# pxl-th/SLAM.jl

Measured on AMD Instinct MI355X. Metric: frames/sec KITTI-05 stereo @1k kpts; local-BA ms/iter for 50-KF window, higher is better.
Workload: dtype f64

## Files before the change

### slam.jl_amd/csrc/kpset.hip

```cpp
#include "kpset.hpp"
#include <algorithm>
#include "geom_device.hpp"
#include "work_order.hpp"
#include "kf_host.hpp"
#include <cmath>
#include <type_traits>

#define WORK_BAND_PX 16
#define KPSET_SORT_LDS_BYTES 65536
static int work_band() { static const int band = [] { const char *v = getenv("SLAMHIP_WORK_BAND"); const int b = v ? atoi(v) : WORK_BAND_PX; return b < 0 ? 0 : b; }(); return band; }
struct WorkOrder { int H, W, band, pad; };
#define SEL_NAME(k) k
#define SEL_ARG
#define SEL_STREAM(b) b
#define SEL_STREAMS(S) S
#define SEL_SELF(s) s
#include "kpset_kernels.inc"
#undef SEL_NAME
#undef SEL_ARG
#undef SEL_STREAM
#undef SEL_STREAMS
#undef SEL_SELF
#define SEL_NAME(k) k##_sel
#define SEL_ARG , const int *sel
#define SEL_STREAM(b) sel[b]
#define SEL_STREAMS(S) (int)gridDim.x
#define SEL_SELF(s) (int)blockIdx.x
#include "kpset_kernels.inc"
#undef SEL_NAME
#undef SEL_ARG
#undef SEL_STREAM
#undef SEL_STREAMS
#undef SEL_SELF

int kpset_build_worklist(slam_ctx *ctx, slam_kpset *ks, int H, int W, bool selected)
{
    WorkOrder O;
    O.H = H; O.W = W; O.pad = ks->sort_pad; O.band = H > 0 && W > 0 && ks->sort_pad > 0 ? work_band() : 0;
    const size_t lds = O.band > 0 ? (size_t)ks->sort_pad * 8 : 0;
    if (selected && ks->n_sel != KPSEL_ALL)
        hipLaunchKernelGGL(k_kpset_worklist_sel, dim3(ks->n_sel), dim3(256), lds, ctx->stream, (const int *)ks->v.count, ks->S, ks->v.cap, ks->work, ks->ntot, (const double *)ks->v.yx, O,
                           (const int *)ks->sel_idx);
    else
        hipLaunchKernelGGL(k_kpset_worklist, dim3(ks->S), dim3(256), lds, ctx->stream, (const int *)ks->v.count, ks->S, ks->v.cap, ks->work, ks->ntot, (const double *)ks->v.yx, O);
    HIP_TRY(ctx, hipGetLastError());
    return SLAM_OK;
}

int kpset_stage_params(slam_ctx *ctx, slam_kpset *ks, const double *host, size_t n, const double **dev_out)
{
    const size_t slot_d = (size_t)ks->S * KP_PAR;
    ARG_TRY(ctx, n <= slot_d);
    const int sl = ks->par_slot; ks->par_slot = (sl + 1) & 7;
    HIP_TRY(ctx, hipEventSynchronize(ks->par_ev[sl]));
    double *h = ks->par_host + (size_t)sl * slot_d, *dv = ks->par + (size_t)sl * slot_d;
    memcpy(h, host, n * 8);
    HIP_TRY(ctx, hipMemcpyAsync(dv, h, n * 8, hipMemcpyHostToDevice, ctx->stream));
    HIP_TRY(ctx, hipEventRecord(ks->par_ev[sl], ctx->stream));
    *dev_out = dv;
    return SLAM_OK;
}

int kpset_compact(slam_ctx *ctx, slam_kpset *ks, int mode, const uint8_t *flags_dev, bool selected)
{
    if (selected && ks->n_sel != KPSEL_ALL)
        hipLaunchKernelGGL(k_kpset_compact_sel, dim3(ks->n_sel), dim3(256), 0, ctx->stream, ks->v, mode, flags_dev, (const int *)ks->sel_idx);
    else
        hipLaunchKernelGGL(k_kpset_compact, dim3(ks->S), dim3(256), 0, ctx->stream, ks->v, mode, flags_dev);
    HIP_TRY(ctx, hipGetLastError());
    return SLAM_OK;
}

struct KTriArgs {
    TwoViewMats M;
    const double *Twc;
    double max_error, min_depth;
};
__device__ __forceinline__ void k_kpset_triangulate_slot(const KpsetView &K, const KTriArgs &T, const int *work, int i)
{
    const size_t q = (size_t)work[i];
    if (!K.stereo[q] || K.is3d[q]) return;
    const int s = (int)(q / K.cap);
    const double x1 = K.yx[2 * q + 1], y1 = K.yx[2 * q], x2 = K.syx[2 * q + 1], y2 = K.syx[2 * q];
    double L[4];
    dlt_two_view(x1, y1, x2, y2, T.M.P1, T.M.P2, L);
    const bool ok = two_view_gates(L, T.M.T21, T.M.cam1, T.M.cam2, x1, y1, x2, y2, T.max_error, T.min_depth, true);
    if (ok) {
        const double *W = T.Twc + 16 * (size_t)s;
        for (int r = 0; r < 3; r++) K.xyz[3 * q + r] = ((W[r] * L[0] + W[r + 4] * L[1]) + W[r + 8] * L[2]) + W[r + 12] * L[3];
        K.is3d[q] = 1;
    } else K.stereo[q] = 0;
}
__global__ __launch_bounds__(64) void k_kpset_triangulate(KpsetView K, KTriArgs T, const int *work, const int *ntot)
{
    const int n = ntot[0];
    for (int i = blockIdx.x * 64 + threadIdx.x; i < n; i += gridDim.x * 64) k_kpset_triangulate_slot(K, T, work, i);
}

struct KTempArgs {
    const double *par;
    const double *tab;
    const int *kf_cur, *kf_lo; int nkf;
    double max_error, min_depth, min_parallax;
    uint8_t *flags;
};
__device__ __forceinline__ void k_kpset_tri_temporal_slot(const KpsetView &K, const KTempArgs &T, const int *work, int i)
{
    const size_t q = (size_t)work[i];
    if (K.is3d[q] || !K.haskf[q]) return;
    const int s = (int)(q / K.cap), kf = K.fkf[q];
    if (kf == T.kf_cur[s] || kf < T.kf_lo[s]) return;
    const double *par = T.par + KP_PAR * (size_t)s, *cam = par + KP_PAR_CAM, *dist = par + KP_PAR_DIST;
    const double *E = T.tab + ((size_t)s * T.nkf + (kf % T.nkf)) * 64;
    const double *P2 = E, *T21 = E + 16, *REL = E + 32, *WOB = E + 48;
    const double fx = cam[0], fy = cam[1], cx = cam[2], cy = cam[3];
    double y1, x1, y2, x2, qy, qx;
    undistort_px(cam, dist, K.fyx[2 * q], K.fyx[2 * q + 1], y1, x1);
    undistort_px(cam, dist, K.yx[2 * q], K.yx[2 * q + 1], y2, x2);
    rotate_project<4>(REL, cam, (x2 - cx) / fx, (y2 - cy) / fy, qy, qx);
    const double pdy = y1 - qy, pdx = x1 - qx;
    const bool gated = sqrt(pdy * pdy + pdx * pdx) > T.min_parallax;
    const double P1[16] = {fx, 0, 0, 0, 0, fy, 0, 0, cx, cy, 1, 0, 0, 0, 0, 1};
    double L[4];
    dlt_two_view(x1, y1, x2, y2, P1, P2, L);
    const bool ok = two_view_gates(L, T21, cam, cam, x1, y1, x2, y2, T.max_error, T.min_depth, gated);
    if (ok) {
        for (int r = 0; r < 3; r++) K.xyz[3 * q + r] = ((WOB[r] * L[0] + WOB[r + 4] * L[1]) + WOB[r + 8] * L[2]) + WOB[r + 12] * L[3];
// ... 90 lines not shown
    double cam[4], dist[4];
    load_cam(par, cam, dist);
    const double fx = cam[0], fy = cam[1], cx = cam[2], cy = cam[3];
    const bool comp = (A.flags & 1) != 0, only2d = (A.flags & 2) != 0;
    for (int w = tid; w < A.words; w += 256) s_bits[w] = 0;
    if (tid == 0) s_base = 0;
    int c[4] = {0, 0, 0, 0};
    for (int j = tid; j < n; j += 256) {
        const bool f3 = A.is3d[b + j] != 0, fk = A.haskf[b + j] != 0;
        c[0] += f3; c[1] += A.stereo[b + j] != 0; c[2] += fk; c[3] += fk && !(only2d && f3);
    }
    kf_block_sum4(c, s_c);
    const int m = c[3];
    const bool in_lds = m <= KF_TERMS_LDS;
    unsigned long long *gterm = A.terms ? A.terms + b : nullptr;
    const double ylim = (double)A.gr * (double)A.cell, xlim = (double)A.gc * (double)A.cell, low = -(double)A.cell;
    double psum = 0.0;
    int isnan_any = 0;
    for (int c0 = 0; c0 < n; c0 += 256) {
        const int j = c0 + tid;
        bool take = false;
        double y = 0.0, x = 0.0;
        if (j < n) {
            y = A.yx[2 * (b + j)]; x = A.yx[2 * (b + j) + 1];
            const double ry = rint(y), rx = rint(x);
            if (ry > low && ry < ylim && rx > low && rx < xlim) {
                const int cell = ((int)ry / A.cell) * A.gc + (int)rx / A.cell;
                atomicOr(&s_bits[cell >> 5], 1u << (cell & 31));
            }
            take = A.haskf[b + j] != 0 && !(only2d && A.is3d[b + j] != 0);
        }
        const int pos = ordered_slot(take, s_w, &s_base);
        if (take) {
            const size_t q = b + j;
            double uy, ux, vy, vx, qy, qx, t;
            undistort_px(cam, dist, y, x, uy, ux);
            undistort_px(cam, dist, A.kyx[2 * q], A.kyx[2 * q + 1], vy, vx);
            if (comp) {
                rotate_project<3>(par, cam, (ux - cx) / fx, (uy - cy) / fy, qy, qx);
                const double dy = qy - vy, dx = qx - vx;
                t = sqrt(dy * dy + dx * dx);
            } else {
                const double dy = uy - vy, dx = ux - vx;
                t = sqrt(dy * dy + dx * dx);
            }
            psum += t;
            isnan_any |= t != t;
            const unsigned long long bits = (unsigned long long)__double_as_longlong(t);
            if (in_lds) s_term[pos] = bits; else gterm[pos] = bits;
        }
    }
    for (int o = 32; o > 0; o >>= 1) psum += __shfl_xor(psum, o, 64);
    if (lane == 0) s_par[wv] = psum;
    __threadfence_block();
    const int has_nan = __syncthreads_or(isnan_any);
    int occ[4] = {0, 0, 0, 0};
    for (int w = tid; w < A.words; w += 256) occ[0] += __popc(s_bits[w]);
    kf_block_sum4(occ, s_c);
    double median = 0.0;
    if (m > 0) {
        if (has_nan) median = __longlong_as_double(0x7FF8000000000000ll);
        else median = in_lds ? kf_median(s_term, m, s_hist, s_w, s_sel, s_min) : kf_median(gterm, m, s_hist, s_w, s_sel, s_min);
    }
    if (tid == 0) {
        double *o = A.out + SLAM_KF_STATS * (size_t)z;
        o[KF_N] = (double)n; o[KF_N3D] = (double)c[0]; o[KF_NSTEREO] = (double)c[1]; o[KF_NHASKF] = (double)c[2]; o[KF_CELLS] = (double)occ[0]; o[KF_NPAR] = (double)m;
        o[KF_MEAN] = m > 0 ? ((s_par[0] + s_par[1]) + (s_par[2] + s_par[3])) / (double)m : 0.0;
        o[KF_MEDIAN] = median;
    }
}

static size_t kpset_regions(slam_kpset *ks, char *base)
{
    Layout Lo;
    auto region = [&](auto *&p, size_t bytes) { const size_t at = Lo.take(bytes); if (base) p = (std::remove_reference_t<decltype(p)>)(base + at); };
    KpsetView &v = ks->v;
    const size_t S = (size_t)ks->S, n = S * v.cap;
    region(v.yx, n * 16); region(v.oyx, n * 16); region(v.syx, n * 16); region(v.xyz, n * 24); region(v.id, n * 8);
    region(v.is3d, n); region(v.stereo, n); region(v.st, n); region(v.count, S * 4); region(ks->work, n * 4); region(ks->ntot, 64);
    region(ks->next_id, S * 8); region(ks->par, 8 * S * KP_PAR * 8); region(v.kyx, n * 16); region(v.haskf, n); region(v.fyx, n * 16);
    region(v.fkf, n * 4); region(v.kfcount, S * 4);
    region(ks->sel_idx, S * 4 + S);
    if (base) ks->sel_mask = (uint8_t *)(ks->sel_idx + S);
    return Lo.size();
}

struct KpField { void *dev; size_t bytes; const void *host; };
static int kpset_copy(slam_ctx *ctx, const slam_kpset *ks, int s, int n, hipMemcpyKind kind, bool wait, std::initializer_list<KpField> fields)
{
    if (n <= 0) return SLAM_OK;
    for (const KpField &f : fields) {
        if (!f.host) continue;
        void *d = (char *)f.dev + (size_t)s * ks->v.cap * f.bytes, *h = const_cast<void *>(f.host);
        HIP_TRY(ctx, hipMemcpyAsync(kind == hipMemcpyHostToDevice ? d : h, kind == hipMemcpyHostToDevice ? h : d, (size_t)n * f.bytes, kind, ctx->stream));
    }
    if (wait) HIP_TRY(ctx, slam_stream_wait(ctx->stream));
    return SLAM_OK;
}
static int kpset_download_begin(slam_ctx *ctx, slam_kpset *ks, int s, const char *who, int cap_out, int *n_out, bool with_kf, int *kf_count)
{
    HIP_TRY(ctx, hipSetDevice(ctx->device));
    int n = 0, kc = 0;
    HIP_TRY(ctx, hipMemcpyAsync(&n, ks->v.count + s, 4, hipMemcpyDeviceToHost, ctx->stream));
    if (with_kf) HIP_TRY(ctx, hipMemcpyAsync(&kc, ks->v.kfcount + s, 4, hipMemcpyDeviceToHost, ctx->stream));
    HIP_TRY(ctx, slam_stream_wait(ctx->stream));
    *n_out = n; if (kf_count) *kf_count = kc;
    if (n > cap_out) return slam_fail(ctx, SLAM_ERR_CAPACITY, "%s: %d keypoints but cap = %d", who, n, cap_out);
    return SLAM_OK;
}

int kpset_read_back(slam_ctx *ctx, char *h, std::initializer_list<KpReadBack> parts)
{
    for (const KpReadBack &p : parts) HIP_TRY(ctx, hipMemcpyAsync(h + p.at, p.dev, p.bytes, hipMemcpyDeviceToHost, ctx->stream));
    HIP_TRY(ctx, slam_stream_wait(ctx->stream));
    for (const KpReadBack &p : parts) if (p.out) memcpy(p.out, h + p.at, p.bytes);
    return SLAM_OK;
}

extern "C" {

int slam_kpset_destroy(slam_kpset *ks);

int slam_kpset_create(slam_ctx *ctx, int S, int cap, slam_kpset **out)
{
    ARG_TRY(ctx, ctx != nullptr && out != nullptr && S >= 1 && S <= 128 && cap >= 1 && (size_t)S * cap < (1u << 30));
    HIP_TRY(ctx, hipSetDevice(ctx->device));
    slam_kpset *ks = new slam_kpset();
    ks->device = ctx->device; ks->S = S; ks->v.cap = cap;
    const size_t bytes = kpset_regions(ks, nullptr);
    { size_t pad = 1; while (pad < (size_t)cap) pad <<= 1; ks->sort_pad = work_band() > 0 && pad * 8 <= KPSET_SORT_LDS_BYTES ? (int)pad : 0; }
    hipError_t e = hipMalloc((void **)&ks->base, bytes);
    if (e == hipSuccess) e = hipMemsetAsync(ks->base, 0, bytes, ctx->stream);
    if (e == hipSuccess) e = slam_stream_wait(ctx->stream);
    if (e != hipSuccess) { if (ks->base) (void)hipFree(ks->base); delete ks; return slam_fail(ctx, SLAM_ERR_HIP, "slam_kpset_create: %s", hipGetErrorString(e)); }
    kpset_regions(ks, ks->base);
    e = hipHostMalloc((void **)&ks->par_host, (size_t)8 * S * KP_PAR * 8);
    for (int i = 0; i < 8 && e == hipSuccess; i++) { e = hipEventCreateWithFlags(&ks->par_ev[i], hipEventDisableTiming); if (e == hipSuccess) e = hipEventRecord(ks->par_ev[i], ctx->stream); }
    if (e != hipSuccess) { slam_kpset_destroy(ks); return slam_fail(ctx, SLAM_ERR_HIP, "slam_kpset_create: %s", hipGetErrorString(e)); }
    *out = ks;
    return SLAM_OK;
}

int slam_kpset_destroy(slam_kpset *ks)
{
    if (!ks) return SLAM_OK;
    (void)hipSetDevice(ks->device);
    (void)hipDeviceSynchronize();
    if (ks->base) (void)hipFree(ks->base);
    if (ks->par_host) (void)hipHostFree(ks->par_host);
    if (ks->kf_stats) (void)hipFree(ks->kf_stats);
    if (ks->kf_terms) (void)hipFree(ks->kf_terms);
    for (int i = 0; i < 8; i++) if (ks->par_ev[i]) (void)hipEventDestroy(ks->par_ev[i]);
    if (ks->sel_pin) (void)hipHostFree(ks->sel_pin);
    for (int i = 0; i < 8; i++) if (ks->sel_ev[i]) (void)hipEventDestroy(ks->sel_ev[i]);
    delete ks;
    return SLAM_OK;
}

int slamhip_test_kpset_worklist(slam_ctx *ctx, slam_kpset *ks, int H, int W, int *work_out, int *ntot_out, int *band_out)
{
    ARG_TRY(ctx, ctx != nullptr && ks != nullptr && work_out != nullptr && ntot_out != nullptr && band_out != nullptr);
    HIP_TRY(ctx, hipSetDevice(ctx->device));
    int rc = kpset_build_worklist(ctx, ks, H, W);
    if (rc) return rc;
    HIP_TRY(ctx, hipMemcpyAsync(work_out, ks->work, (size_t)ks->S * ks->v.cap * 4, hipMemcpyDeviceToHost, ctx->stream));
    HIP_TRY(ctx, hipMemcpyAsync(ntot_out, ks->ntot, 4, hipMemcpyDeviceToHost, ctx->stream));
// ... 233 lines not shown
```

### slam.jl_amd/csrc/kpset.hpp

```cpp
#pragma once
#include "common.hpp"
#include "kpset_select.hpp"
#include <initializer_list>

struct KpsetView {
    double *yx;
    double *oyx;
    double *syx;
    double *xyz;
    double *kyx;
    double *fyx;
    int64_t *id;
    uint8_t *is3d, *stereo, *st, *haskf;
    int *fkf;
    int *kfcount;
    int *count;
    int cap;
};

constexpr int KP_PAR = 32, KP_PAR_CAM = 16, KP_PAR_DIST = 20, KP_PAR_SHIFT = 24;
__device__ __forceinline__ void load_cam(const double *par, double *cam, double *dist) { for (int k = 0; k < 4; k++) { cam[k] = par[KP_PAR_CAM + k]; dist[k] = par[KP_PAR_DIST + k]; } }

struct slam_kpset {
    int device = 0, S = 0;
    char *base = nullptr;
    KpsetView v = {};
    int *work = nullptr;
    int sort_pad = 0;
    int *ntot = nullptr;
    int64_t *next_id = nullptr;
    double *par = nullptr, *par_host = nullptr;
    hipEvent_t par_ev[8] = {};
    int par_slot = 0;
    double *kf_stats = nullptr;
    unsigned long long *kf_terms = nullptr;
    int n_sel = KPSEL_ALL;
    int *sel_idx = nullptr; uint8_t *sel_mask = nullptr;
    uint8_t sel_host[128] = {};
    char *sel_pin = nullptr;
    hipEvent_t sel_ev[8] = {};
    int sel_slot = 0;
};

int kpset_stage_params(slam_ctx *ctx, slam_kpset *ks, const double *host, size_t n, const double **dev_out);
int kpset_build_worklist(slam_ctx *ctx, slam_kpset *ks, int H, int W, bool selected = false);
int kpset_compact(slam_ctx *ctx, slam_kpset *ks, int mode, const uint8_t *flags_dev, bool selected = false);
inline bool kpset_none_selected(const slam_kpset *ks) { return ks->n_sel == 0; }
inline int kpset_sel_streams(const slam_kpset *ks) { return kpset_select_streams(ks->S, ks->n_sel); }
inline const int *kpset_sel_table(const slam_kpset *ks) { return ks->n_sel == KPSEL_ALL ? nullptr : ks->sel_idx; }
inline int kpset_grid_bound(const slam_kpset *ks, int n_bound) { const int nmax = ks->S * ks->v.cap; return n_bound > 0 && n_bound < nmax ? n_bound : nmax; }
inline int kpset_sel_grid_bound(const slam_kpset *ks, int n_bound) { return kpset_select_bound(ks->S, ks->v.cap, ks->n_sel, n_bound); }
struct KpReadBack { size_t at; const void *dev; size_t bytes; void *out; };
int kpset_read_back(slam_ctx *ctx, char *h, std::initializer_list<KpReadBack> parts);
```

### slam.jl_amd/csrc/kpset_kernels.inc

```

__global__ __launch_bounds__(256) void SEL_NAME(k_kpset_worklist)(const int *count, int S, int cap, int *work, int *ntot, const double *yx, WorkOrder O SEL_ARG)
{
    extern __shared__ unsigned long long s_word[];
    const int s = SEL_STREAM(blockIdx.x), tid = threadIdx.x, lane = tid & 63;
    int off = 0, t = 0;
    for (int i = lane; i < SEL_STREAMS(S); i += 64) { const int v = count[SEL_STREAM(i)]; t += v; off += i < SEL_SELF(s) ? v : 0; }
#pragma unroll
    for (int m = 32; m >= 1; m >>= 1) { off += __shfl_xor(off, m); t += __shfl_xor(t, m); }
    if (SEL_SELF(s) == 0 && tid == 0) ntot[0] = t;
    const int n = count[s];
    if (O.band <= 0 || n > O.pad) {
        for (int j = tid; j < n; j += 256) work[off + j] = s * cap + j;
        return;
    }
    int P = 1;
    while (P < n) P <<= 1;
    const double *p = yx + 2 * (size_t)s * cap;
    for (int j = tid; j < P; j += 256)
        s_word[j] = j < n ? ((unsigned long long)work_key(p[2 * j], p[2 * j + 1], O.H, O.W, O.band) << 32) | (unsigned)j : ~0ull;
    __syncthreads();
    for (int k = 2; k <= P; k <<= 1)
        for (int d = k >> 1; d > 0; d >>= 1) {
            for (int u = tid; u < (P >> 1); u += 256) {
                const int i = ((u & ~(d - 1)) << 1) | (u & (d - 1));
                const unsigned long long a = s_word[i], c = s_word[i + d];
                if ((a > c) == ((i & k) == 0)) { s_word[i] = c; s_word[i + d] = a; }
            }
            __syncthreads();
        }
    for (int j = tid; j < n; j += 256) work[off + j] = s * cap + (int)(unsigned)s_word[j];
}

__global__ __launch_bounds__(256) void SEL_NAME(k_kpset_compact)(KpsetView K, int mode, const uint8_t *flags SEL_ARG)
{
    __shared__ int s_w[4], s_base;
    const int s = SEL_STREAM(blockIdx.x), tid = threadIdx.x, lane = tid & 63, wv = tid >> 6;
    const size_t b = (size_t)s * K.cap;
    const int n = K.count[s];
    if (tid == 0) s_base = 0;
    __syncthreads();
    for (int c0 = 0; c0 < n; c0 += 256) {
        const int j = c0 + tid;
        bool keep = false;
        double y = 0, x = 0, sy = 0, sx = 0, X0 = 0, X1 = 0, X2 = 0, ky = 0, kx = 0, fy0 = 0, fx0 = 0; int64_t id = 0; uint8_t f3 = 0, fs = 0, fk = 0; int fkid = 0;
        if (j < n) {
            const size_t q = b + j;
            if (mode == 0) { const uint8_t t = K.st[q]; keep = t != 0; if (t == 1) { y = K.oyx[2 * q]; x = K.oyx[2 * q + 1]; } else { y = K.yx[2 * q]; x = K.yx[2 * q + 1]; } }
            else { keep = flags[q] == 0; y = K.yx[2 * q]; x = K.yx[2 * q + 1]; }
            if (keep) { sy = K.syx[2 * q]; sx = K.syx[2 * q + 1]; X0 = K.xyz[3 * q]; X1 = K.xyz[3 * q + 1]; X2 = K.xyz[3 * q + 2]; id = K.id[q]; f3 = K.is3d[q]; fs = K.stereo[q];
                        ky = K.kyx[2 * q]; kx = K.kyx[2 * q + 1]; fk = K.haskf[q]; fy0 = K.fyx[2 * q]; fx0 = K.fyx[2 * q + 1]; fkid = K.fkf[q]; }
        }
        const unsigned long long m = __ballot(keep);
        const int rank = __builtin_popcountll(m & ((1ull << lane) - 1ull));
        if (lane == 0) s_w[wv] = __builtin_popcountll(m);
        __syncthreads();
        int wbase = 0;
        for (int i = 0; i < wv; i++) wbase += s_w[i];
        const int total = s_w[0] + s_w[1] + s_w[2] + s_w[3];
        if (keep) {
            const size_t q = b + s_base + wbase + rank;
            K.yx[2 * q] = y; K.yx[2 * q + 1] = x; K.syx[2 * q] = sy; K.syx[2 * q + 1] = sx;
            K.xyz[3 * q] = X0; K.xyz[3 * q + 1] = X1; K.xyz[3 * q + 2] = X2; K.id[q] = id; K.is3d[q] = f3; K.stereo[q] = fs;
            K.kyx[2 * q] = ky; K.kyx[2 * q + 1] = kx; K.haskf[q] = fk; K.fyx[2 * q] = fy0; K.fyx[2 * q + 1] = fx0; K.fkf[q] = fkid;
        }
        __syncthreads();
        if (tid == 0) s_base += total;
        __syncthreads();
    }
    if (tid == 0) K.count[s] = s_base;
}

extern "C" __global__ __launch_bounds__(256) void SEL_NAME(k_kpset_keyframe)(KpsetView K SEL_ARG)
{
    const int s = SEL_STREAM(blockIdx.y), j = blockIdx.x * 256 + threadIdx.x;
    if (j >= K.count[s]) return;
    const size_t q = (size_t)s * K.cap + j;
    const double y = K.yx[2 * q], x = K.yx[2 * q + 1];
    if (!K.haskf[q]) { K.fyx[2 * q] = y; K.fyx[2 * q + 1] = x; K.fkf[q] = K.kfcount[s]; }
    K.kyx[2 * q] = y; K.kyx[2 * q + 1] = x; K.haskf[q] = 1;
}
```

### slam.jl_amd/csrc/lk.hip

```cpp
#include "kpset.hpp"
#include "geom_device.hpp"
#include "work_order.hpp"
#include <vector>
#include <cmath>
#include <cstdlib>
#include <type_traits>

struct LKTune {
    int pyramid_levels, levels3d, window, iterations;
    double eig_thr, eps, max_distance;
    bool nonneg() const { return pyramid_levels >= 0 && levels3d >= 0 && window >= 0 && iterations >= 0; }
};
struct LKArgs {
    PyrView prev, cur;
    const double *pts, *disp0;
    int n;
    LKTune tune;
    double *out;
    uint8_t *status;
};

#ifdef LK_TRACE
__device__ unsigned long long g_lk_ticks[8];
#define LKT_BEGIN unsigned long long _t0 = wall_clock64()
// ... 318 lines not shown
    double qy = py, qx = px, cy = dy, cx = dx;
    for (int k = 0; k <= pyramid_levels + 1; k++) {
        const bool back = k == pyramid_levels + 1;
        const int level = back ? 1 : pyramid_levels + 1 - k;
        if (back) {
            ny = py + cy; nx = px + cx;
            qy = ny; qx = nx;
            cy = -cy * 1.0; cx = -cx * 1.0;
        }
        const PyrView *pf = back ? &cur : &prev, *ps = back ? &prev : &cur;
        const bool ok = lk_level<LK_MAXE, TOL>(shifted(pf->lv[level - 1], back ? offC : offP), shifted(ps->lv[level - 1], back ? offP : offC),
                                          level, qy, qx, cy, cx, t.window, t.iterations, t.eig_thr, back ? 1e-2 : t.eps);
        if (!ok) return false;
    }
    const double b0 = ny + cy, b1 = nx + cx;
    const double d0 = py - b0, d1 = px - b1;
    return !(sqrt(d0 * d0 + d1 * d1) >= t.max_distance);
}

#define LK_XCDS 8
__device__ __forceinline__ int xcd_point(int n)
{
    const int per = (n + LK_XCDS - 1) / LK_XCDS;
    return (int)(blockIdx.x % LK_XCDS) * per + (int)(blockIdx.x / LK_XCDS);
}
static inline unsigned lk_grid(int n) { return (unsigned)((n + LK_XCDS - 1) / LK_XCDS) * LK_XCDS; }

template <int LK_MAXE>
__global__ __launch_bounds__(64) LK_OCC void k_fb_track(LKArgs A)
{
    const int i = xcd_point(A.n);
    if (i >= A.n) return;
    const double py = A.pts[2 * i], px = A.pts[2 * i + 1];
    const double dy = A.disp0 ? A.disp0[2 * i] : 0.0, dx = A.disp0 ? A.disp0[2 * i + 1] : 0.0;
    double ny = nan(""), nx = nan("");
    const bool ok = fb_point<LK_MAXE>(A.prev, A.cur, py, px, dy, dx, A.tune, A.tune.pyramid_levels, ny, nx);
    if ((threadIdx.x & 63) == 0) {
        A.out[2 * i] = ny; A.out[2 * i + 1] = nx;
        A.status[i] = ok ? 1 : 0;
    }
}

struct FlowArgs {
    LKArgs lk;
    const uint8_t *is3d; const double *proj;
    const int *img;
    size_t zs_from, zs_to;
};
template <int LK_MAXE>
__global__ __launch_bounds__(64) LK_OCC void k_flow_match(FlowArgs F)
{
    const LKArgs &A = F.lk;
    const int i = xcd_point(A.n);
    if (i >= A.n) return;
    LKT_BEGIN;
    const double py = A.pts[2 * i], px = A.pts[2 * i + 1];
    double ny = nan(""), nx = nan("");
    bool ok = false;
    const size_t zi = F.img ? (size_t)F.img[i] : 0;
    const size_t offP = zi * F.zs_from, offC = zi * F.zs_to;
    for (int att = F.is3d[i] ? 0 : 1; att < 2 && !ok; att++) {
        double dy = 0.0, dx = 0.0;
        if (att == 0) {
            const double scale = 1.0 / (double)(1 << A.tune.levels3d);
            dy = scale * (F.proj[2 * i] - py); dx = scale * (F.proj[2 * i + 1] - px);
        }
        ok = fb_point<LK_MAXE>(A.prev, A.cur, py, px, dy, dx, A.tune, att == 0 ? A.tune.levels3d : A.tune.pyramid_levels, ny, nx, offP, offC);
    }
    LKT(0);
    if ((threadIdx.x & 63) == 0) {
        A.out[2 * i] = ok ? ny : nan(""); A.out[2 * i + 1] = ok ? nx : nan("");
        A.status[i] = ok ? 1 : 0;
    }
}

struct KpMatchArgs {
    PyrView from, to; size_t zs_from, zs_to;
    LKTune tune;
    double *yx, *oyx, *syx; const double *xyz; const uint8_t *is3d; uint8_t *st, *stereo; int cap;
    const int *work, *ntot;
    int prior;
    const double *par;
    int H, W, stereo_mode; double epipolar;
};
template <int LK_MAXE, bool TOL>
__global__ __launch_bounds__(64) LK_OCC void k_kpset_match(KpMatchArgs M)
{
    const int ntot = M.ntot[0], per = (ntot + LK_XCDS - 1) / LK_XCDS;
    for (int slotx = (int)(blockIdx.x / LK_XCDS); slotx < per; slotx += (int)(gridDim.x / LK_XCDS)) {
    const int idx = (int)(blockIdx.x % LK_XCDS) * per + slotx;
    if (idx >= ntot) break;
    const size_t q = (size_t)M.work[idx];
    const int s = (int)(q / M.cap);
    const double *P = M.par + KP_PAR * (size_t)s, *cam = P + KP_PAR_CAM, *dist = P + KP_PAR_DIST;
    const double py = M.yx[2 * q], px = M.yx[2 * q + 1];
    const bool is3 = M.is3d[q] != 0;
    double pry = py, prx = px;
    if (is3) {
        if (M.prior == 1) {
            const double X0 = M.xyz[3 * q], X1 = M.xyz[3 * q + 1], X2 = M.xyz[3 * q + 2];
            const double cx = ((P[0] * X0 + P[4] * X1) + P[8] * X2) + P[12];
            const double cy = ((P[1] * X0 + P[5] * X1) + P[9] * X2) + P[13];
            const double cz = ((P[2] * X0 + P[6] * X1) + P[10] * X2) + P[14];
            pdn_to_pixel(cam, dist, cy / cz, cx / cz, pry, prx);
        } else if (M.prior == 2) { pry = py + P[KP_PAR_SHIFT]; prx = px + P[KP_PAR_SHIFT + 1]; }
    }
    const bool inside = 1 <= pry && pry <= (double)M.H && 1 <= prx && prx <= (double)M.W;
    const bool lane0 = (threadIdx.x & 63) == 0;
    if (is3 && !inside) {
        if (lane0) { M.st[q] = M.stereo_mode ? 0 : 2; if (M.stereo_mode) M.stereo[q] = 0; }
        continue;
    }
    const size_t offF = (size_t)s * M.zs_from, offT = (size_t)s * M.zs_to;
    double ny = nan(""), nx = nan("");
    bool ok = false;
    for (int att = is3 ? 0 : 1; att < 2 && !ok; att++) {
        double dy = 0.0, dx = 0.0;
        if (att == 0) {
            const double scale = 1.0 / (double)(1 << M.tune.levels3d);
            dy = scale * (pry - py); dx = scale * (prx - px);
        }
        ok = fb_point<LK_MAXE, TOL>(M.from, M.to, py, px, dy, dx, M.tune, att == 0 ? M.tune.levels3d : M.tune.pyramid_levels, ny, nx, offF, offT);
    }
    if (lane0 && !M.stereo_mode) {
        M.oyx[2 * q] = ok ? ny : nan(""); M.oyx[2 * q + 1] = ok ? nx : nan("");
        M.st[q] = ok ? 1 : 0;
    } else if (lane0) {
        if (ok) {
            double uy, ux;
            undistort_px(cam, dist, ny, nx, uy, ux);
            if (fabs(py - uy) > M.epipolar) ok = false;
        }
        if (ok) { M.syx[2 * q] = py; M.syx[2 * q + 1] = nx; }
        M.stereo[q] = ok ? 1 : 0;
        M.st[q] = 2;
    }
    }
}

template <class F> static void lk_launch(int window, F f)
{
    switch (lk_slots(window)) {
    case 3: f(std::integral_constant<int, 3>{}); break;
    case 6: f(std::integral_constant<int, 6>{}); break;
    default: f(std::integral_constant<int, 9>{});
    }
}

static int match_check(slam_ctx *ctx, const slam_pyr *from, const slam_pyr *to, const LKTune &t)
{
    const int need = t.pyramid_levels > t.levels3d ? t.pyramid_levels : t.levels3d;
    if (!(from->levels > need && to->levels > need)) return slam_fail(ctx, SLAM_ERR_LAYERS, "Not enough layers in pyramids.");
    ARG_TRY(ctx, from->H[0] == to->H[0] && from->W[0] == to->W[0]);
    if (from->target_only) return slam_fail(ctx, SLAM_ERR_ARG, "the source pyramid of a match was updated with SLAM_PYR_TARGET_ONLY: its gradient planes exist at level 0 only");
    return SLAM_OK;
}

static int kpset_match(slam_ctx *ctx, slam_kpset *ks, const slam_pyr *from0, const slam_pyr *to0, const double *params,
                       int prior, const LKTune &t, int stereo_mode, double epipolar, int n_bound)
{
    ARG_TRY(ctx, ctx != nullptr && ks != nullptr && from0 != nullptr && to0 != nullptr);
    ARG_TRY(ctx, from0->batch_index == 0 && to0->batch_index == 0 && from0->batch_size >= ks->S && to0->batch_size >= ks->S);
    ARG_TRY(ctx, t.nonneg() && prior >= 0 && prior <= 2 && (prior == 0 || params != nullptr));
    int rc = match_check(ctx, from0, to0, t);
    if (rc) return rc;
    HIP_TRY(ctx, hipSetDevice(ctx->device));
    const bool selected = stereo_mode != 0;
    if (selected && kpset_none_selected(ks)) return SLAM_OK;
    KpMatchArgs M;
    M.from = from0->view; M.to = to0->view; M.zs_from = from0->zstride; M.zs_to = to0->zstride;
    M.tune = t;
    const KpsetView &v = ks->v;
    M.yx = v.yx; M.oyx = v.oyx; M.syx = v.syx; M.xyz = v.xyz; M.is3d = v.is3d; M.st = v.st; M.stereo = v.stereo; M.cap = v.cap;
    M.work = ks->work; M.ntot = ks->ntot; M.prior = prior; M.H = from0->H[0]; M.W = from0->W[0]; M.stereo_mode = stereo_mode; M.epipolar = epipolar;
    std::vector<double> zero;
    if (!params) { zero.assign((size_t)ks->S * KP_PAR, 0.0); for (int s = 0; s < ks->S; s++) { zero[KP_PAR * s + KP_PAR_CAM] = zero[KP_PAR * s + KP_PAR_CAM + 1] = 1.0; } params = zero.data(); }
    rc = kpset_stage_params(ctx, ks, params, (size_t)ks->S * KP_PAR, &M.par);
    if (rc) return rc;
    rc = kpset_build_worklist(ctx, ks, M.H, M.W, selected);
    if (rc) return rc;
    int nb = selected ? kpset_sel_grid_bound(ks, n_bound) : kpset_grid_bound(ks, n_bound);
    static const int grid_cap = [] { const char *v = getenv("SLAMHIP_LK_GRID"); return v ? atoi(v) : 0; }();
    if (grid_cap > 0 && nb > grid_cap) nb = grid_cap;
    { ProfScope span(ctx, "fb_track");
      static const bool no_tol_lk = getenv("SLAMHIP_NO_TOL_LK") != nullptr;
      const bool tol = from0->tol_planes && to0->tol_planes && !no_tol_lk;
      if (tol) lk_launch(t.window, [&](auto N) { hipLaunchKernelGGL((k_kpset_match<N.value, true>), dim3(lk_grid(nb)), dim3(64), 0, ctx->stream, M); });
      else lk_launch(t.window, [&](auto N) { hipLaunchKernelGGL((k_kpset_match<N.value, false>), dim3(lk_grid(nb)), dim3(64), 0, ctx->stream, M); }); }
    HIP_TRY(ctx, hipGetLastError());
    return kpset_compact(ctx, ks, 0, nullptr, selected);
}

extern "C" int slam_kpset_flow_match(slam_ctx *ctx, slam_kpset *ks, const slam_pyr *from0, const slam_pyr *to0, const double *params, int prior,
                                     int pyramid_levels, int pyramid_levels_3d, int window, int iterations, double eig_thr, double eps,
                                     double max_distance, int n_bound)
{
    return kpset_match(ctx, ks, from0, to0, params, prior, {pyramid_levels, pyramid_levels_3d, window, iterations, eig_thr, eps, max_distance}, 0, 0.0, n_bound);
}
extern "C" int slam_kpset_stereo_match(slam_ctx *ctx, slam_kpset *ks, const slam_pyr *left0, const slam_pyr *right0, const double *params, int prior,
                                       int pyramid_levels, int pyramid_levels_3d, int window, int iterations, double eig_thr, double eps,
                                       double max_distance, double epipolar_error, int n_bound)
{
    return kpset_match(ctx, ks, left0, right0, params, prior, {pyramid_levels, pyramid_levels_3d, window, iterations, eig_thr, eps, max_distance}, 1, epipolar_error, n_bound);
}

#define LK_STAGE_MIN_POINTS 4096

struct TrackLists {
    const double *pts, *aux; const uint8_t *is3d; const int32_t *img; int n;
    double *out; uint8_t *status; bool flow;
};

static int run_tracking(slam_ctx *ctx, const slam_pyr *prev, const slam_pyr *cur, const LKTune &t, const TrackLists &l)
{
    const int n = l.n;
    Layout B;
    const size_t o_pts = B.take((size_t)n * 16), o_aux = B.take((size_t)n * 16), o_3d = B.take((size_t)n), o_img = B.take((size_t)n * 4), in_b = B.size();
    const size_t o_out = B.take((size_t)n * 16), o_st = B.take((size_t)n), out_b = B.size() - in_b;
    char *h, *d;
    int rc = slam_pinned(ctx, B.size(), (void **)&h);
    if (rc) return rc;
    HIP_TRY(ctx, hipHostGetDevicePointer((void **)&d, h, 0));
    memcpy(h + o_pts, l.pts, (size_t)n * 16);
    if (l.aux) memcpy(h + o_aux, l.aux, (size_t)n * 16);
    if (l.is3d) memcpy(h + o_3d, l.is3d, (size_t)n);
    if (l.img) memcpy(h + o_img, l.img, (size_t)n * 4);
    const bool staged = n >= LK_STAGE_MIN_POINTS;
    if (staged) {
        void *dbuf;
        rc = slam_scratch(ctx, B.size(), &dbuf);
        if (rc) return rc;
        HIP_TRY(ctx, hipMemcpyAsync(dbuf, h, in_b, hipMemcpyHostToDevice, ctx->stream));
        d = (char *)dbuf;
    }
    FlowArgs F;
    LKArgs &A = F.lk;
    A.prev = prev->view; A.cur = cur->view;
    A.pts = (const double *)(d + o_pts); A.disp0 = l.aux ? (const double *)(d + o_aux) : nullptr; A.n = n;
    A.tune = t;
    A.out = (double *)(d + o_out); A.status = (uint8_t *)(d + o_st);
    F.is3d = (const uint8_t *)(d + o_3d); F.proj = (const double *)(d + o_aux);
    F.img = l.img ? (const int *)(d + o_img) : nullptr; F.zs_from = prev->zstride; F.zs_to = cur->zstride;
    { ProfScope span(ctx, "fb_track");
      if (l.flow) lk_launch(t.window, [&](auto N) { hipLaunchKernelGGL(k_flow_match<N.value>, dim3(lk_grid(n)), dim3(64), 0, ctx->stream, F); });
      else lk_launch(t.window, [&](auto N) { hipLaunchKernelGGL(k_fb_track<N.value>, dim3(lk_grid(n)), dim3(64), 0, ctx->stream, A); }); }
    HIP_TRY(ctx, hipGetLastError());
    if (staged) HIP_TRY(ctx, hipMemcpyAsync(h + in_b, d + in_b, out_b, hipMemcpyDeviceToHost, ctx->stream));
    HIP_TRY(ctx, slam_stream_wait(ctx->stream));
    memcpy(l.out, h + o_out, (size_t)n * 16);
    memcpy(l.status, h + o_st, (size_t)n);
    return SLAM_OK;
}

extern "C" int slam_fb_track(slam_ctx *ctx, const slam_pyr *prev, const slam_pyr *cur,
                             const double *pts_yx, const double *disp0_yx, int n,
                             int pyramid_levels, int window, int iterations,
                             double eig_thr, double eps, double max_distance,
                             double *out_yx, uint8_t *status)
{
    const LKTune t = {pyramid_levels, 0, window, iterations, eig_thr, eps, max_distance};
    ARG_TRY(ctx, ctx != nullptr && prev != nullptr && cur != nullptr);
    ARG_TRY(ctx, n >= 0 && t.nonneg());
    if (n == 0) return SLAM_OK;
// ... 66 lines not shown
```

### slam.jl_amd/csrc/work_order.hpp

```cpp
#pragma once
#include <cstdint>

#if defined(__HIPCC__)
#define WORK_HD __host__ __device__ __forceinline__
#else
#define WORK_HD static inline
#endif

#define WORK_KEY_MAX_PX 65535

WORK_HD uint32_t work_clamp_px(double v, int hi)
{
    const uint32_t top = (uint32_t)(hi < 0 ? 0 : hi > WORK_KEY_MAX_PX ? WORK_KEY_MAX_PX : hi);
    if (v != v) return top;
    if (!(v >= 1.0)) return 0;
    if (v >= (double)top) return top;
    return (uint32_t)v;
}

WORK_HD uint32_t work_key(double y, double x, int H, int W, int band)
{
    return ((work_clamp_px(x, W) / (uint32_t)(band < 1 ? 1 : band)) << 16) | work_clamp_px(y, H);
}

WORK_HD int lk_window_elems(int window) { return (2 * window + 1) * (2 * window + 1); }
WORK_HD int lk_slots(int window) { const int ne = lk_window_elems(window); return ne <= 192 ? 3 : ne <= 384 ? 6 : 9; }
```

Baseline: 24200.

## Precompute per-keypoint match records in worklist build and scalar-load them in LK

The worklist kernel now also writes a 48-byte record per work item, laid out per XCD. Each record holds the position, the projected prior and the flags for that keypoint. The LK match kernel fetches its record with wave-uniform scalar loads (s_load via inline asm), fused with the ntot load, so it no longer does a dependent gather through work, yx, is3d, xyz and par and recomputes the prior per block. The cost is extra record writes and memory, plus inline asm that assumes the record address is uniform and aligned. The change also adds LKT timing hooks and a precomputed scale for the level-3D step.

```diff
diff --git a/slam.jl_amd/csrc/kpset.hip b/slam.jl_amd/csrc/kpset.hip
--- a/slam.jl_amd/csrc/kpset.hip
+++ b/slam.jl_amd/csrc/kpset.hip
@@ -10,6 +10,20 @@
 #define KPSET_SORT_LDS_BYTES 65536
 static int work_band() { static const int band = [] { const char *v = getenv("SLAMHIP_WORK_BAND"); const int b = v ? atoi(v) : WORK_BAND_PX; return b < 0 ? 0 : b; }(); return band; }
 struct WorkOrder { int H, W, band, pad; };
+bool kpset_match_records() { static const bool on = [] { const char *v = getenv("SLAMHIP_NO_MATCH_REC"); return !(v && atoi(v) != 0); }(); return on; }
+__device__ __forceinline__ void kp_write_rec(const KpWorkRecs &R, const double *yx, int H, int W, int idx, int per, int q, int s)
+{
+    const int at = work_rec_slot(idx, per, R.stride);
+    if (at >= WORK_XCDS * R.stride) return;
+    KpWorkRec r;
+    r.py = yx[2 * (size_t)q]; r.px = yx[2 * (size_t)q + 1];
+    const bool is3 = R.is3d[q] != 0;
+    double pry, prx;
+    kp_match_prior(R.prior, R.xyz + 3 * (size_t)q, R.par + KP_PAR * (size_t)s, r.py, r.px, pry, prx);
+    r.pry = is3 ? pry : r.py; r.prx = is3 ? prx : r.px;
+    r.q = q; r.s = s; r.flags = (is3 ? KPREC_3D : 0) | (kp_in_image(r.pry, r.prx, H, W) ? KPREC_INSIDE : 0); r.pad = 0;
+    R.rec[at] = r;
+}
 #define SEL_NAME(k) k
 #define SEL_ARG
 #define SEL_STREAM(b) b
@@ -33,16 +47,18 @@
 #undef SEL_STREAMS
 #undef SEL_SELF
 
-int kpset_build_worklist(slam_ctx *ctx, slam_kpset *ks, int H, int W, bool selected)
+int kpset_build_worklist(slam_ctx *ctx, slam_kpset *ks, int H, int W, bool selected, const KpMatchPrior *match)
 {
     WorkOrder O;
     O.H = H; O.W = W; O.pad = ks->sort_pad; O.band = H > 0 && W > 0 && ks->sort_pad > 0 ? work_band() : 0;
     const size_t lds = O.band > 0 ? (size_t)ks->sort_pad * 8 : 0;
+    KpWorkRecs R = {nullptr, 0, 0, nullptr, nullptr, nullptr};
+    if (match && kpset_match_records()) R = {ks->rec, ks->rec_stride, match->prior, match->par, ks->v.xyz, ks->v.is3d};
     if (selected && ks->n_sel != KPSEL_ALL)
-        hipLaunchKernelGGL(k_kpset_worklist_sel, dim3(ks->n_sel), dim3(256), lds, ctx->stream, (const int *)ks->v.count, ks->S, ks->v.cap, ks->work, ks->ntot, (const double *)ks->v.yx, O,
+        hipLaunchKernelGGL(k_kpset_worklist_sel, dim3(ks->n_sel), dim3(256), lds, ctx->stream, (const int *)ks->v.count, ks->S, ks->v.cap, ks->work, ks->ntot, (const double *)ks->v.yx, O, R,
                            (const int *)ks->sel_idx);
     else
-        hipLaunchKernelGGL(k_kpset_worklist, dim3(ks->S), dim3(256), lds, ctx->stream, (const int *)ks->v.count, ks->S, ks->v.cap, ks->work, ks->ntot, (const double *)ks->v.yx, O);
+        hipLaunchKernelGGL(k_kpset_worklist, dim3(ks->S), dim3(256), lds, ctx->stream, (const int *)ks->v.count, ks->S, ks->v.cap, ks->work, ks->ntot, (const double *)ks->v.yx, O, R);
     HIP_TRY(ctx, hipGetLastError());
     return SLAM_OK;
 }
@@ -299,6 +315,8 @@
     region(v.fkf, n * 4); region(v.kfcount, S * 4);
     region(ks->sel_idx, S * 4 + S);
     if (base) ks->sel_mask = (uint8_t *)(ks->sel_idx + S);
+    ks->rec_stride = work_rec_stride((long long)n);
+    region(ks->rec, (size_t)WORK_XCDS * ks->rec_stride * sizeof(KpWorkRec));
     return Lo.size();
 }
 
diff --git a/slam.jl_amd/csrc/kpset.hpp b/slam.jl_amd/csrc/kpset.hpp
--- a/slam.jl_amd/csrc/kpset.hpp
+++ b/slam.jl_amd/csrc/kpset.hpp
@@ -1,6 +1,7 @@
 #pragma once
 #include "common.hpp"
 #include "kpset_select.hpp"
+#include "geom_device.hpp"
 #include <initializer_list>
 
 struct KpsetView {
@@ -21,6 +22,33 @@
 constexpr int KP_PAR = 32, KP_PAR_CAM = 16, KP_PAR_DIST = 20, KP_PAR_SHIFT = 24;
 __device__ __forceinline__ void load_cam(const double *par, double *cam, double *dist) { for (int k = 0; k < 4; k++) { cam[k] = par[KP_PAR_CAM + k]; dist[k] = par[KP_PAR_DIST + k]; } }
 
+__device__ __forceinline__ void kp_match_prior(int prior, const double *X, const double *P, double py, double px, double &pry, double &prx)
+{
+    pry = py; prx = px;
+    if (prior == 1) {
+        const double X0 = X[0], X1 = X[1], X2 = X[2];
+        const double cx = ((P[0] * X0 + P[4] * X1) + P[8] * X2) + P[12];
+        const double cy = ((P[1] * X0 + P[5] * X1) + P[9] * X2) + P[13];
+        const double cz = ((P[2] * X0 + P[6] * X1) + P[10] * X2) + P[14];
+        pdn_to_pixel(P + KP_PAR_CAM, P + KP_PAR_DIST, cy / cz, cx / cz, pry, prx);
+    } else if (prior == 2) { pry = py + P[KP_PAR_SHIFT]; prx = px + P[KP_PAR_SHIFT + 1]; }
+}
+__device__ __forceinline__ bool kp_in_image(double y, double x, int H, int W) { return 1 <= y && y <= (double)H && 1 <= x && x <= (double)W; }
+
+struct alignas(16) KpWorkRec {
+    double py, px;
+    double pry, prx;
+    int q, s;
+    int flags;
+    int pad;
+};
+constexpr int KPREC_3D = 1, KPREC_INSIDE = 2;
+static_assert(sizeof(KpWorkRec) == 48 && alignof(KpWorkRec) == 16, "the fetch of k_kpset_match (lk.hip) restates the layout");
+struct KpWorkRecs {
+    KpWorkRec *rec; int stride;
+    int prior; const double *par, *xyz; const uint8_t *is3d;
+};
+
 struct slam_kpset {
     int device = 0, S = 0;
     char *base = nullptr;
@@ -28,6 +56,8 @@
     int *work = nullptr;
     int sort_pad = 0;
     int *ntot = nullptr;
+    KpWorkRec *rec = nullptr;
+    int rec_stride = 0;
     int64_t *next_id = nullptr;
     double *par = nullptr, *par_host = nullptr;
     hipEvent_t par_ev[8] = {};
@@ -43,7 +73,9 @@
 };
 
 int kpset_stage_params(slam_ctx *ctx, slam_kpset *ks, const double *host, size_t n, const double **dev_out);
-int kpset_build_worklist(slam_ctx *ctx, slam_kpset *ks, int H, int W, bool selected = false);
+struct KpMatchPrior { int prior; const double *par; };
+bool kpset_match_records();
+int kpset_build_worklist(slam_ctx *ctx, slam_kpset *ks, int H, int W, bool selected = false, const KpMatchPrior *match = nullptr);
 int kpset_compact(slam_ctx *ctx, slam_kpset *ks, int mode, const uint8_t *flags_dev, bool selected = false);
 inline bool kpset_none_selected(const slam_kpset *ks) { return ks->n_sel == 0; }
 inline int kpset_sel_streams(const slam_kpset *ks) { return kpset_select_streams(ks->S, ks->n_sel); }
diff --git a/slam.jl_amd/csrc/kpset_kernels.inc b/slam.jl_amd/csrc/kpset_kernels.inc
--- a/slam.jl_amd/csrc/kpset_kernels.inc
+++ b/slam.jl_amd/csrc/kpset_kernels.inc
@@ -1,5 +1,5 @@
 
-__global__ __launch_bounds__(256) void SEL_NAME(k_kpset_worklist)(const int *count, int S, int cap, int *work, int *ntot, const double *yx, WorkOrder O SEL_ARG)
+__global__ __launch_bounds__(256) void SEL_NAME(k_kpset_worklist)(const int *count, int S, int cap, int *work, int *ntot, const double *yx, WorkOrder O, KpWorkRecs R SEL_ARG)
 {
     extern __shared__ unsigned long long s_word[];
     const int s = SEL_STREAM(blockIdx.x), tid = threadIdx.x, lane = tid & 63;
@@ -8,9 +8,9 @@
 #pragma unroll
     for (int m = 32; m >= 1; m >>= 1) { off += __shfl_xor(off, m); t += __shfl_xor(t, m); }
     if (SEL_SELF(s) == 0 && tid == 0) ntot[0] = t;
-    const int n = count[s];
+    const int n = count[s], per = work_rec_per(t);
     if (O.band <= 0 || n > O.pad) {
-        for (int j = tid; j < n; j += 256) work[off + j] = s * cap + j;
+        for (int j = tid; j < n; j += 256) { work[off + j] = s * cap + j; if (R.rec) kp_write_rec(R, yx, O.H, O.W, off + j, per, s * cap + j, s); }
         return;
     }
     int P = 1;
@@ -28,7 +28,11 @@
             }
             __syncthreads();
         }
-    for (int j = tid; j < n; j += 256) work[off + j] = s * cap + (int)(unsigned)s_word[j];
+    for (int j = tid; j < n; j += 256) {
+        const int q = s * cap + (int)(unsigned)s_word[j];
+        work[off + j] = q;
+        if (R.rec) kp_write_rec(R, yx, O.H, O.W, off + j, per, q, s);
+    }
 }
 
 __global__ __launch_bounds__(256) void SEL_NAME(k_kpset_compact)(KpsetView K, int mode, const uint8_t *flags SEL_ARG)
diff --git a/slam.jl_amd/csrc/lk.hip b/slam.jl_amd/csrc/lk.hip
--- a/slam.jl_amd/csrc/lk.hip
+++ b/slam.jl_amd/csrc/lk.hip
@@ -424,43 +424,72 @@
     int prior;
     const double *par;
     int H, W, stereo_mode; double epipolar;
+    const KpWorkRec *rec; int rec_stride, use_rec;
 };
+__device__ __forceinline__ KpWorkRec load_rec_uniform(const KpWorkRec *p)
+{
+    typedef int rec_v4i __attribute__((ext_vector_type(4)));
+    const __attribute__((address_space(4))) rec_v4i *c = (const __attribute__((address_space(4))) rec_v4i *)p;
+    const rec_v4i a = c[0], b = c[1], d = c[2];
+    KpWorkRec r;
+    r.py = __hiloint2double(a.y, a.x); r.px = __hiloint2double(a.w, a.z);
+    r.pry = __hiloint2double(b.y, b.x); r.prx = __hiloint2double(b.w, b.z);
+    r.q = d.x; r.s = d.y; r.flags = d.z; r.pad = 0;
+    return r;
+}
+__device__ __forceinline__ KpWorkRec load_rec_and_ntot(const KpWorkRec *p, const int *ntot_p, int &ntot)
+{
+    typedef int rec_v4i __attribute__((ext_vector_type(4)));
+    typedef int rec_v8i __attribute__((ext_vector_type(8)));
+    rec_v8i a; rec_v4i d;
+    asm volatile("s_load_dwordx8 %0, %3, 0x0\n\ts_load_dwordx4 %1, %3, 0x20\n\ts_load_dword %2, %4, 0x0\n\ts_waitcnt lgkmcnt(0)"
+                 : "=&s"(a), "=&s"(d), "=&s"(ntot) : "s"(p), "s"(ntot_p) : "memory");
+    KpWorkRec r;
+    r.py = __hiloint2double(a[1], a[0]); r.px = __hiloint2double(a[3], a[2]);
+    r.pry = __hiloint2double(a[5], a[4]); r.prx = __hiloint2double(a[7], a[6]);
+    r.q = d[0]; r.s = d[1]; r.flags = d[2]; r.pad = 0;
+    return r;
+}
 template <int LK_MAXE, bool TOL>
 __global__ __launch_bounds__(64) LK_OCC void k_kpset_match(KpMatchArgs M)
 {
-    const int ntot = M.ntot[0], per = (ntot + LK_XCDS - 1) / LK_XCDS;
-    for (int slotx = (int)(blockIdx.x / LK_XCDS); slotx < per; slotx += (int)(gridDim.x / LK_XCDS)) {
-    const int idx = (int)(blockIdx.x % LK_XCDS) * per + slotx;
+    LKT_BEGIN;
+    const int xcd = (int)(blockIdx.x % LK_XCDS), slot0 = (int)(blockIdx.x / LK_XCDS);
+    int ntot;
+    KpWorkRec rc = load_rec_and_ntot(M.rec + ((size_t)xcd * M.rec_stride + slot0), M.ntot, ntot);
+    const int per = (ntot + LK_XCDS - 1) / LK_XCDS;
+    for (int slotx = slot0; slotx < per; slotx += (int)(gridDim.x / LK_XCDS)) {
+    const int idx = xcd * per + slotx;
     if (idx >= ntot) break;
-    const size_t q = (size_t)M.work[idx];
-    const int s = (int)(q / M.cap);
+    size_t q; int s; double py, px, pry, prx; bool is3, inside;
+    const double scale3 = __hiloint2double((1023 - M.tune.levels3d) << 20, 0);
+    if (M.use_rec) {
+        if (slotx != slot0) rc = load_rec_uniform(M.rec + ((size_t)xcd * M.rec_stride + slotx));
+        q = (size_t)rc.q; s = rc.s; py = rc.py; px = rc.px; pry = rc.pry; prx = rc.prx;
+        is3 = (rc.flags & KPREC_3D) != 0; inside = (rc.flags & KPREC_INSIDE) != 0;
+    } else {
+        q = (size_t)M.work[idx];
+        s = (int)(q / M.cap);
+        py = M.yx[2 * q]; px = M.yx[2 * q + 1];
+        is3 = M.is3d[q] != 0;
+        pry = py; prx = px;
+        if (is3) kp_match_prior(M.prior, M.xyz + 3 * q, M.par + KP_PAR * (size_t)s, py, px, pry, prx);
+        inside = kp_in_image(pry, prx, M.H, M.W);
+    }
     const double *P = M.par + KP_PAR * (size_t)s, *cam = P + KP_PAR_CAM, *dist = P + KP_PAR_DIST;
-    const double py = M.yx[2 * q], px = M.yx[2 * q + 1];
-    const bool is3 = M.is3d[q] != 0;
-    double pry = py, prx = px;
-    if (is3) {
-        if (M.prior == 1) {
-            const double X0 = M.xyz[3 * q], X1 = M.xyz[3 * q + 1], X2 = M.xyz[3 * q + 2];
-            const double cx = ((P[0] * X0 + P[4] * X1) + P[8] * X2) + P[12];
-            const double cy = ((P[1] * X0 + P[5] * X1) + P[9] * X2) + P[13];
-            const double cz = ((P[2] * X0 + P[6] * X1) + P[10] * X2) + P[14];
-            pdn_to_pixel(cam, dist, cy / cz, cx / cz, pry, prx);
-        } else if (M.prior == 2) { pry = py + P[KP_PAR_SHIFT]; prx = px + P[KP_PAR_SHIFT + 1]; }
-    }
-    const bool inside = 1 <= pry && pry <= (double)M.H && 1 <= prx && prx <= (double)M.W;
     const bool lane0 = (threadIdx.x & 63) == 0;
     if (is3 && !inside) {
         if (lane0) { M.st[q] = M.stereo_mode ? 0 : 2; if (M.stereo_mode) M.stereo[q] = 0; }
         continue;
     }
+    LKT(6);
     const size_t offF = (size_t)s * M.zs_from, offT = (size_t)s * M.zs_to;
     double ny = nan(""), nx = nan("");
     bool ok = false;
     for (int att = is3 ? 0 : 1; att < 2 && !ok; att++) {
         double dy = 0.0, dx = 0.0;
         if (att == 0) {
-            const double scale = 1.0 / (double)(1 << M.tune.levels3d);
-            dy = scale * (pry - py); dx = scale * (prx - px);
+            dy = scale3 * (pry - py); dx = scale3 * (prx - px);
         }
         ok = fb_point<LK_MAXE, TOL>(M.from, M.to, py, px, dy, dx, M.tune, att == 0 ? M.tune.levels3d : M.tune.pyramid_levels, ny, nx, offF, offT);
     }
@@ -477,6 +506,7 @@
         M.stereo[q] = ok ? 1 : 0;
         M.st[q] = 2;
     }
+    LKT(7);
     }
 }
 
@@ -519,8 +549,10 @@
     if (!params) { zero.assign((size_t)ks->S * KP_PAR, 0.0); for (int s = 0; s < ks->S; s++) { zero[KP_PAR * s + KP_PAR_CAM] = zero[KP_PAR * s + KP_PAR_CAM + 1] = 1.0; } params = zero.data(); }
     rc = kpset_stage_params(ctx, ks, params, (size_t)ks->S * KP_PAR, &M.par);
     if (rc) return rc;
-    rc = kpset_build_worklist(ctx, ks, M.H, M.W, selected);
+    const KpMatchPrior mp = {prior, M.par};
+    rc = kpset_build_worklist(ctx, ks, M.H, M.W, selected, &mp);
     if (rc) return rc;
+    M.rec = ks->rec; M.rec_stride = ks->rec_stride; M.use_rec = kpset_match_records() ? 1 : 0;
     int nb = selected ? kpset_sel_grid_bound(ks, n_bound) : kpset_grid_bound(ks, n_bound);
     static const int grid_cap = [] { const char *v = getenv("SLAMHIP_LK_GRID"); return v ? atoi(v) : 0; }();
     if (grid_cap > 0 && nb > grid_cap) nb = grid_cap;
diff --git a/slam.jl_amd/csrc/work_order.hpp b/slam.jl_amd/csrc/work_order.hpp
--- a/slam.jl_amd/csrc/work_order.hpp
+++ b/slam.jl_amd/csrc/work_order.hpp
@@ -23,5 +23,11 @@
     return ((work_clamp_px(x, W) / (uint32_t)(band < 1 ? 1 : band)) << 16) | work_clamp_px(y, H);
 }
 
+#define WORK_XCDS 8
+WORK_HD int work_rec_stride(long long slots) { return (int)((slots + WORK_XCDS - 1) / WORK_XCDS); }
+WORK_HD int work_rec_per(int ntot) { return (ntot + WORK_XCDS - 1) / WORK_XCDS; }
+WORK_HD int work_rec_slot(int idx, int per, int stride) { return (idx / per) * stride + idx % per; }
+WORK_HD int work_rec_entry(int x, int r, int per, int ntot) { return r < per && x * per + r < ntot ? x * per + r : -1; }
+
 WORK_HD int lk_window_elems(int window) { return (2 * window + 1) * (2 * window + 1); }
 WORK_HD int lk_slots(int window) { const int ne = lk_window_elems(window); return ne <= 192 ? 3 : ne <= 384 ? 6 : 9; }
```

Result: faster. 24610 (median of 6 runs) (+1.7%).
